# lcp29/trimesh-ray-optix

Measured on AMD Instinct MI355X. Metric: Mrays/s closest-hit, 1M-tri mesh, 1024^2 ray batch, higher is better.
Workload: dtype f32; 1 GPU; C5(i): icosphere(8)+displacement seed 0, 1310720 tris; 1024x1024 pinhole rays per GPU; intersects_closest (stream_compaction=False); rays_per_gpu=1048576, rays_total=1048576, triangles=1310720, parallelism=ray-sharded x1, BVH replicated, warmup_steps_done=368, bvh_depth=30, bvh_bytes=104857568

## Files before the change

### include/triro_hip.h

```cpp
#ifndef TRIRO_HIP_H
#define TRIRO_HIP_H

#include <stdint.h>

#ifdef __cplusplus
extern "C" {
#endif

#define TR_ABI_VERSION 10
#define TR_MAX_ANYHIT_SIZE 8
#define TR_MAX_SIZE_LENGTH 4
#define TR_MAX_HITS_CAP 32

typedef enum tr_status {
    TR_OK = 0,
    TR_ERR_INVALID_ARG = 1,
    TR_ERR_HIP = 2,
    TR_ERR_NO_DEVICE = 3,
    TR_ERR_OUT_OF_MEMORY = 4,
    TR_ERR_INTERNAL = 5
} tr_status;

typedef struct tr_bvh tr_bvh;

// ... 55 lines not shown
int tr_bvh_serialize(const tr_bvh *bvh, void *h_buffer, int64_t size, void *stream);
int tr_bvh_deserialize(const void *h_buffer, int64_t size, void *stream, tr_bvh **out);
int tr_bvh_get_info(const tr_bvh *bvh, tr_bvh_info *info);
int tr_bvh_last_launch(const tr_bvh *bvh, tr_launch_info *info);

typedef struct tr_topology {
    int32_t num_cus, num_xcd, waves_per_cu, reserved;
    int64_t l2_bytes;
    int64_t resident_lanes;
    int64_t steal_max_rays, wide_min_rays, count_stream_min_rays;
} tr_topology;
int tr_device_topology(int device, tr_topology *out);
int tr_bvh_download(const tr_bvh *bvh, void *h_nodes, void *h_links, void *h_tris,
                    void *stream);
int tr_bvh_download_qnodes(const tr_bvh *bvh, void *h_qnodes, float *h_frame6, void *stream);

int tr_intersects_any(const tr_bvh *bvh, const tr_rays *rays, uint8_t *d_hit, void *stream);
int tr_intersects_first(const tr_bvh *bvh, const tr_rays *rays, int32_t *d_tri, void *stream);
int tr_intersects_closest(const tr_bvh *bvh, const tr_rays *rays, uint8_t *d_hit,
                          uint8_t *d_front, int32_t *d_tri, float *d_loc, float *d_uv,
                          void *stream);
int tr_intersects_count(const tr_bvh *bvh, const tr_rays *rays, int32_t *d_count, void *stream);

typedef struct tr_packed_hit {
    uint32_t tri;
    float w0, w1;
} tr_packed_hit;
int tr_intersects_closest_packed(const tr_bvh *bvh, const tr_rays *rays, tr_packed_hit *d_packed,
                                 void *stream);
int tr_closest_expand(const tr_packed_hit *d_packed, int64_t n, const float *d_vertices, int64_t nv,
// ... 54 lines not shown
```

### trimesh-ray-optix_amd/csrc/api.hip

```cpp
#include <atomic>
#include <mutex>
#include <string.h>

#include "tr_internal.h"

namespace {
thread_local std::string g_last_error;
std::mutex g_mutex;
constexpr int TR_MAX_DEVICES = 64;
tr_device_state g_devices[TR_MAX_DEVICES];

struct opt_desc {
    const char* name;
    int tr_options::*field;
    int64_t lo, hi;
    bool boolean;
};
const opt_desc OPTS[] = {
    {"adaptive", &tr_options::adaptive, 0, 1, true},
    {"compact", &tr_options::compact, 0, 1, true},
    {"xcd_chunk", &tr_options::xcd_chunk, 0, 65536, false},
    {"steal", &tr_options::steal, 0, 4096, false},
    {"tile", &tr_options::tile, 0, 2, false},
    {"tile_small", &tr_options::tile_small, 0, 4, false},
// ... 250 lines not shown
    if (hipGetDevice(&device) != hipSuccess)
        return tr_fail(TR_ERR_NO_DEVICE, "no HIP device available (libtriro_hip has no CPU fallback)");
    tr_device_state* st;
    TR_TRY(tr_get_device_state(device, &st));
    tr_bvh* bvh = handle_new(device);
    if (!bvh) return tr_fail(TR_ERR_OUT_OF_MEMORY, "host allocation failed");
    int s = tr_build_impl(bvh, nullptr, 0, nullptr, 0, (hipStream_t)stream);
    if (s == TR_OK && h.num_tris > 0) {
        s = tr_arena_alloc(bvh, h.num_tris);
        if (s == TR_OK && tr_arena_used_bytes(h.num_tris) != h.arena_bytes) s = tr_fail(TR_ERR_INVALID_ARG, "arena size mismatch");
        if (s == TR_OK) {
            if (hipMemcpyAsync(bvh->arena, (const char*)h_buffer + sizeof h, (size_t)h.arena_bytes, hipMemcpyHostToDevice, (hipStream_t)stream) != hipSuccess ||
                hipStreamSynchronize((hipStream_t)stream) != hipSuccess)
                s = tr_fail(TR_ERR_HIP, "upload of the BVH arena failed");
        }
        if (s == TR_OK) {
            bvh->num_tris = h.num_tris; bvh->num_nodes = h.num_nodes; bvh->depth = h.depth; bvh->key_mode = h.key_mode;
            for (int k = 0; k < 3; k++) { bvh->aabb_min[k] = h.aabb_min[k]; bvh->aabb_max[k] = h.aabb_max[k]; }
            tr_qframe_make(bvh->aabb_min, bvh->aabb_max, &bvh->frame);
            s = tr_bvh_sync_frame(bvh);
        }
    }
    if (s != TR_OK) return handle_discard(bvh, s);
    *out = bvh;
    return TR_OK;
}

int tr_bvh_destroy(tr_bvh* bvh) {
    if (!bvh) return TR_OK;
    int status = TR_OK;
    {
        tr_device_guard g;
        if (g.enter(bvh->device) == TR_OK) {
            if (bvh->arena && hipFree(bvh->arena) != hipSuccess) status = tr_fail(TR_ERR_HIP, "hipFree(arena)");
            if (bvh->refit_temp && hipFree(bvh->refit_temp) != hipSuccess) status = tr_fail(TR_ERR_HIP, "hipFree(refit_temp)");
            if (bvh->frame_dev && hipFree(bvh->frame_dev) != hipSuccess) status = tr_fail(TR_ERR_HIP, "hipFree(frame_dev)");
            if (bvh->wnodes && hipFree(bvh->wnodes) != hipSuccess) status = tr_fail(TR_ERR_HIP, "hipFree(wnodes)");
            if (bvh->wflag && hipFree(bvh->wflag) != hipSuccess) status = tr_fail(TR_ERR_HIP, "hipFree(wflag)");
            if (bvh->widx && hipFree(bvh->widx) != hipSuccess) status = tr_fail(TR_ERR_HIP, "hipFree(widx)");
            if (bvh->wide_event) (void)hipEventDestroy(bvh->wide_event);
            for (int k = 0; k < TR_SCHED_SLOTS; k++) {
                if (bvh->sched[k].buf && hipFree(bvh->sched[k].buf) != hipSuccess) status = tr_fail(TR_ERR_HIP, "hipFree(sched)");
                if (bvh->sched[k].wspill && hipFree(bvh->sched[k].wspill) != hipSuccess) status = tr_fail(TR_ERR_HIP, "hipFree(wspill)");
            }
        }
    }
    delete bvh->sched_mutex;
    delete bvh;
    return status;
}

// ... 59 lines not shown
}

int tr_bvh_download_qnodes(const tr_bvh* bvh, void* h_qnodes, float* h_frame6, void* stream) {
    if (!bvh) return tr_fail(TR_ERR_INVALID_ARG, "bvh == NULL");
    hipStream_t s = (hipStream_t)stream;
    tr_device_guard g;
    TR_TRY(tr_enter_device(&g, bvh->device));
    if (h_qnodes && bvh->num_nodes)
        TR_HIP_TRY(hipMemcpyAsync(h_qnodes, bvh->qnodes, sizeof(tr_qnode) * (size_t)bvh->num_nodes, hipMemcpyDeviceToHost, s));
    TR_HIP_TRY(hipStreamSynchronize(s));
    if (h_frame6)
        for (int k = 0; k < 3; k++) { h_frame6[k] = bvh->frame.base[k]; h_frame6[3 + k] = bvh->frame.scale[k]; }
    return TR_OK;
}

int tr_bvh_download(const tr_bvh* bvh, void* h_nodes, void* h_links, void* h_tris, void* stream) {
    if (!bvh) return tr_fail(TR_ERR_INVALID_ARG, "bvh == NULL");
    hipStream_t s = (hipStream_t)stream;
    tr_device_guard g;
    TR_TRY(tr_enter_device(&g, bvh->device));
    if (h_nodes && bvh->num_nodes)
        TR_HIP_TRY(hipMemcpyAsync(h_nodes, bvh->nodes, sizeof(tr_node) * (size_t)bvh->num_nodes, hipMemcpyDeviceToHost, s));
    if (h_links && bvh->num_nodes)
        TR_HIP_TRY(hipMemcpyAsync(h_links, bvh->links, sizeof(tr_link) * (size_t)bvh->num_nodes, hipMemcpyDeviceToHost, s));
    if (h_tris && bvh->num_tris)
        TR_HIP_TRY(hipMemcpyAsync(h_tris, bvh->tris, sizeof(tr_tri) * (size_t)bvh->num_tris, hipMemcpyDeviceToHost, s));
    TR_HIP_TRY(hipStreamSynchronize(s));
    return TR_OK;
}

// ... 19 lines not shown
```

### trimesh-ray-optix_amd/csrc/bvh_build.hip

```cpp
#include <string.h>

#include "tr_internal.h"
#include "tr_lbvh.h"

namespace {

constexpr int RS_KPT = 16;
constexpr int RS_TILE = 64 * RS_KPT;
constexpr int RS_WAVES = 4;

__device__ __forceinline__ uint32_t enc_f32(float f) {
    uint32_t b = __float_as_uint(f);
    return (b & 0x80000000u) ? ~b : (b | 0x80000000u);
}
__device__ __forceinline__ float dec_f32(uint32_t e) {
    uint32_t b = (e & 0x80000000u) ? (e & 0x7fffffffu) : ~e;
    return __uint_as_float(b);
}

__global__ void k_init_bounds(uint32_t* bounds) {
    int t = threadIdx.x;
    if (t < 3) bounds[t] = 0xffffffffu;
    else if (t < 6) bounds[t] = 0u;
    else if (t == 6) bounds[6] = 0xffffffffu;
// ... 260 lines not shown
__global__ void k_qframe(const uint32_t* __restrict__ bounds, tr_qframe* __restrict__ frame) {
    if (threadIdx.x != 0 || blockIdx.x != 0) return;
    float mn[3], mx[3];
    for (int k = 0; k < 3; k++) { mn[k] = dec_f32(bounds[k]); mx[k] = dec_f32(bounds[3 + k]); }
    tr_qframe f;
    tr_qframe_make(mn, mx, &f);
    *frame = f;
}
__global__ void k_qframe_box(const float* __restrict__ box, tr_qframe* __restrict__ frame) {
    if (threadIdx.x != 0 || blockIdx.x != 0) return;
    tr_qframe f;
    tr_qframe_make(box, box + 3, &f);
    *frame = f;
}

__global__ __launch_bounds__(256) void k_emit(const int32_t* __restrict__ childL,
                                              const int32_t* __restrict__ childR,
                                              const int32_t* __restrict__ parent,
                                              const float* __restrict__ sbox,
                                              const float* __restrict__ ibox, int64_t ninternal,
                                              const tr_qframe* __restrict__ frame,
                                              const int32_t* __restrict__ pos,
                                              tr_node* __restrict__ nodes,
                                              tr_link* __restrict__ links,
                                              tr_qnode* __restrict__ qnodes) {
    int64_t i = (int64_t)blockIdx.x * blockDim.x + threadIdx.x;
    if (i >= ninternal) return;
    int32_t cl = childL[i], cr = childR[i];
    const float* a = cl < 0 ? sbox + 6 * (int64_t)(~cl) : ibox + 6 * (int64_t)cl;
    const float* b = cr < 0 ? sbox + 6 * (int64_t)(~cr) : ibox + 6 * (int64_t)cr;
    tr_node nd;
    tr_node_set_box(nd.box0, a, a + 3);
    tr_node_set_box(nd.box1, b, b + 3);
    int32_t p = parent[i];
    int32_t sib = 0;
    if (p >= 0) sib = (childL[p] == (int32_t)i) ? childR[p] : childL[p];
    if (pos && pos[i] < 0) return;
    if (pos) {
        if (cl >= 0) cl = pos[cl];
        if (cr >= 0) cr = pos[cr];
        if (p >= 0) { if (sib >= 0) sib = pos[sib]; p = pos[p]; }
// ... 50 lines not shown
    const float* b = cr < 0 ? sbox + 6 * (int64_t)(~cr) : ibox + 6 * (int64_t)cr;
    float* o = ibox + 6 * i;
#pragma unroll
    for (int k = 0; k < 3; k++) {
        o[k] = fminf(a[k], b[k]);
        o[3 + k] = fmaxf(a[3 + k], b[3 + k]);
    }
    ready[i] = round;
}

__global__ __launch_bounds__(256) void k_update_boxes(tr_node* __restrict__ nodes,
                                                      const float* __restrict__ sbox,
                                                      const float* __restrict__ ibox,
                                                      int64_t ninternal,
                                                      const tr_qframe* __restrict__ frame,
                                                      tr_qnode* __restrict__ qnodes) {
    int64_t i = (int64_t)blockIdx.x * blockDim.x + threadIdx.x;
    if (i >= ninternal) return;
    const int32_t cl = nodes[i].c0, cr = nodes[i].c1;
    const float* a = cl < 0 ? sbox + 6 * (int64_t)(~cl) : ibox + 6 * (int64_t)cl;
    const float* b = cr < 0 ? sbox + 6 * (int64_t)(~cr) : ibox + 6 * (int64_t)cr;
    tr_node_set_box(nodes[i].box0, a, a + 3);
    tr_node_set_box(nodes[i].box1, b, b + 3);
    const tr_qframe f = *frame;
    tr_qnode_set_box(qnodes[i].q, a, a + 3, f);
    tr_qnode_set_box(qnodes[i].q + 3, b, b + 3, f);
}

inline int64_t cdiv(int64_t a, int64_t b) { return (a + b - 1) / b; }
inline size_t align_up(size_t x, size_t a) { return (x + a - 1) / a * a; }

struct Carver {
// ... 26 lines not shown
        TR_HIP_TRY(hipMalloc(&fresh, bytes));
        if (bvh->arena) (void)hipFree(bvh->arena);
        bvh->arena = fresh;
        bvh->arena_bytes = (int64_t)bytes;
        bvh->capacity_tris = nf;
    }
    carve_arena(bvh, (char*)bvh->arena, nf);
    return TR_OK;
}

int64_t tr_arena_used_bytes(int64_t nf) { return (int64_t)carve_arena(nullptr, nullptr, nf); }

int tr_bvh_sync_frame(tr_bvh* bvh) {
    if (!bvh->frame_dev) TR_HIP_TRY(hipMalloc((void**)&bvh->frame_dev, sizeof(tr_qframe)));
    TR_HIP_TRY(hipMemcpy(bvh->frame_dev, &bvh->frame, sizeof(tr_qframe), hipMemcpyHostToDevice));
    return TR_OK;
}

void tr_bvh_reset(tr_bvh* bvh) {
    bvh->wide_valid = false; bvh->wide_unavailable = false;
    bvh->frame = tr_qframe{{0.f, 0.f, 0.f}, {1.f, 1.f, 1.f}};
    bvh->num_tris = 0; bvh->num_nodes = 0; bvh->depth = 0; bvh->key_mode = 0;
    for (int k = 0; k < 3; k++) { bvh->aabb_min[k] = 0.f; bvh->aabb_max[k] = 0.f; }
    for (int k = 0; k < TR_SCHED_SLOTS; k++) { bvh->sched[k].nblocks = 0; }
}

constexpr int TB = 256;
constexpr uint32_t NO_FACE = 0xffffffffu;

static void check(int* status, hipError_t e, const char* what) {
// ... 115 lines not shown
    int32_t root_ready = 0;
    int32_t round = 0;
    const int32_t max_rounds = 160;
    int32_t batch = guess;
    while (root_ready == 0 && round < max_rounds && *status == TR_OK) {
        for (int k = 0; k < batch; k++) {
            ++round;
            hipLaunchKernelGGL(k_refit_round, dim3(gI), dim3(TB), 0, stream, t.cl, t.cr, t.sbox, t.ibox, t.ready, ni, round);
        }
        check(status, hipGetLastError(), "k_refit_round");
        if (!lay_joined) { check(status, hipStreamWaitEvent(stream, st->build_join, 0), "join layout"); lay_joined = true; }
        while (treelets && lround * TR_TREELET_LEVELS < round + TR_TREELET_LEVELS) {
            ++lround;
            hipLaunchKernelGGL(k_layout_round, dim3(gI), dim3(TB), 0, stream, t.cl, t.cr, t.span, t.lpos, t.lbase, t.lflag, ni, lround);
        }
        hipLaunchKernelGGL(k_emit, dim3(gI), dim3(TB), 0, stream, t.cl, t.cr, t.par, t.sbox, t.ibox, ni, t.frame,
                           treelets ? t.lpos : nullptr, bvh->nodes, bvh->links, bvh->qnodes);
        check(status, hipGetLastError(), "k_emit");
        check(status, hipMemcpyAsync(&root_ready, t.ready, sizeof(int32_t), hipMemcpyDeviceToHost, stream), "memcpy root");
        check(status, hipStreamSynchronize(stream), "sync refit");
        if (*bad_face != NO_FACE) return 0;
        batch = 8;
    }
    return root_ready;
}

static void build_hierarchy(tr_bvh* bvh, tr_device_state* st, const build_temps& t, int64_t nf, bool treelets,
                            const uint32_t* bad_face, hipStream_t stream, int* status) {
    int32_t guess = bvh->depth > 0 ? bvh->depth + 1 : 10;
    if (bvh->depth <= 0) for (int64_t m = 1; m < nf; m <<= 1) ++guess;
    if (guess > 64) guess = 64;
    bvh->depth = 0;
// ... 4 lines not shown
        bvh->depth = height;
        bvh->key_mode = mode;
        if (height <= 64) return;
        if (mode == 1) *status = tr_fail(TR_ERR_INTERNAL, "tree height > 64 with bounded keys");
    }
}

int tr_build_impl(tr_bvh* bvh, const float* d_vertices, int64_t nv, const int32_t* d_faces,
                  int64_t nf, hipStream_t stream) {
    if (nf < 0 || nv < 0) return tr_fail(TR_ERR_INVALID_ARG, "negative mesh size");
    if (nf >= (int64_t)1 << 31) return tr_fail(TR_ERR_INVALID_ARG, "more than 2^31-1 triangles");
    bvh->wide_valid = false; bvh->wide_unavailable = false;
    if (nf > 0 && (!d_faces || (!d_vertices && nv > 0))) return tr_fail(TR_ERR_INVALID_ARG, "null mesh pointer");

    int status = tr_arena_alloc(bvh, nf);
    if (status == TR_OK) {
        bvh->num_tris = nf;
        bvh->num_nodes = nf >= 2 ? nf - 1 : 0;
        bvh->depth = 0;
        bvh->key_mode = 0;
        for (int k = 0; k < TR_SCHED_SLOTS; k++) { bvh->sched[k].launches = 0; }
        for (int k = 0; k < 3; k++) { bvh->aabb_min[k] = 0.f; bvh->aabb_max[k] = 0.f; }
    }
    tr_device_state* st = nullptr;
    build_temps t;
    void* temp = nullptr;
    if (status == TR_OK && nf > 0) status = tr_get_device_state(bvh->device, &st);
    if (status == TR_OK && nf > 0) status = tr_build_temp_acquire(st, carve_build_temps(&t, nullptr, nf), &temp);
    if (status == TR_OK && nf > 0) {
        carve_build_temps(&t, (char*)temp, nf);
// ... 54 lines not shown
    }
    carve_refit_temps(&t, (char*)bvh->refit_temp, nf, ni);
    tr_qframe* d_frame = reinterpret_cast<tr_qframe*>(t.bad + 4);
    uint32_t hbad = NO_FACE;
    int status = TR_OK;
    check(&status, hipMemsetAsync(t.bad, 0xff, sizeof(uint32_t), stream), "memset bad-face word");
    hipLaunchKernelGGL(k_regather, dim3((unsigned)cdiv(nf, TB)), dim3(TB), 0, stream, d_vertices, nv, d_faces, nf, bvh->tris, t.sbox, t.bad);
    check(&status, hipGetLastError(), "k_regather");
    check(&status, hipMemcpyAsync(&hbad, t.bad, sizeof(uint32_t), hipMemcpyDeviceToHost, stream), "memcpy bad-face word");
    if (ni > 0) {
        const unsigned gI = (unsigned)cdiv(ni, TB);
        check(&status, hipMemsetAsync(t.ready, 0, sizeof(int32_t) * (size_t)ni, stream), "memset ready");
        for (int32_t round = 1; round <= bvh->depth; round++)
            hipLaunchKernelGGL(k_refit_nodes_round, dim3(gI), dim3(TB), 0, stream, bvh->nodes, t.sbox, t.ibox, t.ready, ni, round);
        hipLaunchKernelGGL(k_qframe_box, dim3(1), dim3(64), 0, stream, t.ibox, d_frame);
        hipLaunchKernelGGL(k_update_boxes, dim3(gI), dim3(TB), 0, stream, bvh->nodes, t.sbox, t.ibox, ni, d_frame, bvh->qnodes);
        check(&status, hipGetLastError(), "refit rounds");
    }
    float box[6];
    check(&status, hipMemcpyAsync(box, ni > 0 ? t.ibox : t.sbox, sizeof(box), hipMemcpyDeviceToHost, stream),
          ni > 0 ? "memcpy root box" : "memcpy box");
    check(&status, hipStreamSynchronize(stream), "sync refit");
    if (status == TR_OK) status = set_bounds(bvh, box, box + 3);
    if (status == TR_OK && hbad != NO_FACE) status = bad_face(hbad, nv);
    return status == TR_OK ? TR_OK : fail_reset(bvh, status);
}
```

### trimesh-ray-optix_amd/csrc/kernels_direct.inc

```
template <bool C, bool DEEP = false> struct tr_word { typedef uint64_t T; };
template <> struct tr_word<true, false> { typedef uint32_t T; };

constexpr bool TR_STREAM_QN = true;
template <int Q> constexpr bool TR_STREAM_COLD = Q != TR_Q_CLOSEST;
template <int Q, int K, bool STATS, bool COMPACT = false, bool UNI = false, bool DEEP = false>
__device__ __forceinline__ void wave_traverse(const tr_bvh_view& b, tr_ray& r, bool go,
                                              tr_result& res, tr_topk<K>& top, tr_counters* cnt,
                                              const tr_ring ring) {
    tr_result_init(res);
    if (Q == TR_Q_LOCATION) top.init();
    typedef typename tr_word<COMPACT, DEEP>::T W;
    tr_state_t<W> fs;
    tr_state_init(fs);
    if (!go) fs.node = -1;
    while (!tr_done(fs)) {
        tr_fused_step<Q, K, STATS, COMPACT, W, UNI, true>(b, r, fs, res, top, cnt, ring);
        TR_CONVERGE();
        tr_fused_step<Q, K, STATS, COMPACT, W, UNI, false>(b, r, fs, res, top, cnt, ring);
        TR_CONVERGE();
    }
}

constexpr uint32_t TR_STEAL_EVERY = 3u;
constexpr uint32_t TR_STEAL_EARLY = 4u;
// ... 74 lines not shown
    if constexpr (PLAIN) {
        bool l0 = false, l1 = false;
        int32_t c0 = 0, c1 = 0;
        bool stop = false;
        {
            const unsigned long long act = __ballot(go);
            if (act != 0ull && trip < steal_min) {
                const int first = (int)__builtin_ctzll(act);
                const uint32_t sn = (uint32_t)__builtin_amdgcn_readlane((int)r.sel_n, first);
                const uint32_t sf = (uint32_t)__builtin_amdgcn_readlane((int)r.sel_f, first);
                const uint32_t sz = (uint32_t)__builtin_amdgcn_readlane((int)r.sel_z, first);
                if (__ballot(go && (r.sel_n != sn || r.sel_f != sf || r.sel_z != sz)) == 0ull) {
                    const tr_uoctant oct = tr_uniform_octant(sn, sz);
                    int32_t nu = 0;
                    tr_uwave u;
                    bool more;
#pragma unroll 1
                    do {
                        typedef const __attribute__((address_space(4))) int32_t* tr_ci32p;
                        const tr_ci32p sp = (tr_ci32p)(unsigned long long)tr_qnode_ptr<COMPACT>(b, nu);
                        tr_i4 w0, w1;
                        w0.x = sp[0]; w0.y = sp[1]; w0.z = sp[2]; w0.w = sp[3];
                        w1.x = sp[4]; w1.y = sp[5]; w1.z = sp[6]; w1.w = sp[7];
                        bool a0, a1, lt;
                        tr_uniform_test<Q>(r, w0, w1, oct, res, a0, a1, lt);
                        if (STATS && go) cnt->nodes++;
                        u = tr_uniform_wave(act, __builtin_amdgcn_ballot_w64(a0), __builtin_amdgcn_ballot_w64(a1),
                                            __builtin_amdgcn_ballot_w64(lt), w1.z, w1.w);
                        c0 = w1.z; c1 = w1.w;
                        if (tr_lane_in(u.both, lane)) tr_addr_push(ar, fs.sa, tr_lane_in(u.sw, lane) ? c0 : c1);
                        TR_CONVERGE();
                        trip++;
                        more = ((u.l0 | u.l1 | u.pop) == 0ull) & ((u.sw == 0ull) | (u.sw == act)) & (trip < steal_min);
                        nu = u.sw != 0ull ? c1 : c0;
                    } while (more);
                    l0 = tr_lane_in(u.l0, lane); l1 = tr_lane_in(u.l1, lane);
                    if (go) fs.node = tr_lane_in(u.sw, lane) ? c1 : c0;
                    if (tr_lane_in(u.pop, lane)) fs.node = tr_addr_pop(ar, fs.sa);
                    stop = (u.l0 | u.l1) != 0ull || !TR_WAVE_ANY(fs.node >= 0);
                }
            }
        }
        if (!stop) while (trip < steal_min) {
            l0 = false; l1 = false;
            if (fs.node >= 0) tr_descent_step<Q, STATS, COMPACT>(b, r, fs, res, cnt, ring, l0, l1, c0, c1);
            TR_CONVERGE();
            trip++;
            if (TR_WAVE_ANY(l0 || l1) || !TR_WAVE_ANY(fs.node >= 0)) break;
        }
        fs.p0 = l0 ? ~c0 : (l1 ? ~c1 : -1);
// ... 705 lines not shown
```

### trimesh-ray-optix_amd/csrc/tr_bvh.h

```cpp
#pragma once
#include <type_traits>
#include "tr_math.h"
#include "../../include/triro_hip.h"

struct alignas(16) tr_f4 {
    float x, y, z, w;
};
struct alignas(16) tr_i4 {
    int32_t x, y, z, w;
};

struct alignas(64) tr_node {
    float box0[6];
    float box1[6];
    int32_t c0, c1;
    int32_t parent;
    int32_t sibling;
};
static_assert(sizeof(tr_node) == 64, "node must be 64 B");
TR_HD void tr_node_set_box(float* box, const float* lo, const float* hi) {
    box[0] = lo[0]; box[1] = lo[1]; box[2] = lo[2]; box[3] = hi[2]; box[4] = hi[0]; box[5] = hi[1];
}

struct alignas(8) tr_link {
// ... 110 lines not shown
    float ax, ay, az, bx, by, bz, cx, cy, cz;
    int32_t face;
    float esum;
    int32_t pad1;
};
static_assert(sizeof(tr_tri) == 48, "tri record must be 48 B");

struct tr_bvh_view {
    const tr_node* nodes;
    const tr_link* links;
    const tr_tri* tris;
    int64_t num_tris;
    const tr_qnode* qnodes;
    tr_qframe frame;
    const tr_qframe* frame_dev;
};
#if defined(__HIP_DEVICE_COMPILE__)
#define TR_VIEW_LIVE(b) do { if ((b).frame_dev) (b).frame = *(b).frame_dev; } while (0)
#else
#define TR_VIEW_LIVE(b) ((void)0)
#endif
enum tr_query { TR_Q_ANY = 0, TR_Q_FIRST = 1, TR_Q_CLOSEST = 2, TR_Q_COUNT = 3, TR_Q_LOCATION = 4 };

struct tr_counters {
    uint32_t nodes, tris, climbs;
};

template <int K>
struct tr_topk {
    float t[K];
// ... 726 lines not shown
    u.l1 = m1 ^ h1;
    u.both = h0 & h1;
    u.sw = ((u.both & lt) | ~h0) & act;
    u.pop = act & ~(h0 | h1);
    return u;
}
TR_HD bool tr_lane_in(uint64_t mask, int lane) {
#if defined(__HIP_DEVICE_COMPILE__)
    (void)lane;
    return __builtin_amdgcn_inverse_ballot_w64(mask);
#else
    return ((mask >> lane) & 1ull) != 0ull;
#endif
}


constexpr int TR_LEAFQ = 6;
struct tr_leafq {
    int32_t* base;
    int32_t stride;
};

template <typename W>
struct tr_ustate_t {
    int32_t node;
    uint32_t depth;
    W trail, owned;
    int32_t nq;
    int32_t pe;
};
// ... 108 lines not shown
```

### trimesh-ray-optix_amd/csrc/tr_internal.h

```cpp
#pragma once
#include <hip/hip_runtime.h>
#include <stdint.h>
#include <mutex>
#include <string>

#include "../../include/triro_hip.h"
#include "tr_bvh.h"
#include "tr_wide.h"

void tr_set_error(const std::string& msg);
int tr_fail(int code, const std::string& msg);

#define TR_HIP_TRY(expr)                                                                  \
    do {                                                                                  \
        hipError_t _e = (expr);                                                           \
        if (_e != hipSuccess) {                                                           \
            return tr_fail(_e == hipErrorOutOfMemory ? TR_ERR_OUT_OF_MEMORY : TR_ERR_HIP, \
                           std::string(#expr) + ": " + hipGetErrorName(_e) + " (" +       \
                               hipGetErrorString(_e) + ")");                              \
        }                                                                                 \
    } while (0)

#define TR_TRY(expr)            \
    do {                        \
// ... 26 lines not shown
struct tr_bvh {
    int device = 0;
    int64_t num_tris = 0;
    int64_t num_nodes = 0;
    int32_t depth = 0;
    int32_t key_mode = 0;
    void* arena = nullptr;
    int64_t arena_bytes = 0;
    int64_t capacity_tris = 0;
    tr_node* nodes = nullptr;
    tr_link* links = nullptr;
    tr_tri* tris = nullptr;
    tr_qnode* qnodes = nullptr;
    tr_qframe frame = {{0, 0, 0}, {1, 1, 1}};
    tr_qframe* frame_dev = nullptr;
    float aabb_min[3] = {0, 0, 0};
    float aabb_max[3] = {0, 0, 0};
    void* refit_temp = nullptr;
    size_t refit_temp_bytes = 0;
    tr_sched_slot sched[TR_SCHED_SLOTS];
    std::mutex* sched_mutex = nullptr;
    tr_wnode* wnodes = nullptr;
    int64_t wcap = 0, wcount = 0;
    uint8_t* wflag = nullptr;
    int64_t* widx = nullptr;
    int64_t wtmp_cap = 0;
    bool wide_valid = false;
    bool wide_unavailable = false;
    hipEvent_t wide_event = nullptr;
    hipStream_t wide_stream = nullptr;
    tr_launch_info last_launch = {};
    bool have_last_launch = false;
};

inline tr_bvh_view tr_view_of(const tr_bvh* bvh) {
    tr_bvh_view view;
    view.nodes = bvh->nodes; view.links = bvh->links; view.tris = bvh->tris; view.num_tris = bvh->num_tris;
    view.qnodes = bvh->qnodes; view.frame = bvh->frame; view.frame_dev = bvh->frame_dev;
    return view;
}

int tr_bvh_sync_frame(tr_bvh* bvh);

struct tr_device_state {
    bool ready = false;
    int device = 0;
    int num_cus = 0;
    int num_xcd = 8;
    int64_t l2_bytes = 0;
    int waves_per_cu = 0;
    int* counters = nullptr;
    unsigned next_counter = 0;
    void* build_temp = nullptr;
    size_t build_temp_bytes = 0;
    std::mutex build_mutex;
// ... 87 lines not shown
```

### trimesh-ray-optix_amd/triro/backend/ops.py

```python
from __future__ import annotations

import ctypes as C
import os
from typing import Tuple

import torch

_INT64_MAX = (1 << 63) - 1
MAX_ANYHIT_SIZE = 8
MAX_SIZE_LENGTH = 4

_LIB_NAME = "libtriro_hip.so"
ABI_VERSION = 10
_lib = None
_lib_error = None


class TrRays(C.Structure):
    _fields_ = [("d_origins", C.c_void_p), ("d_directions", C.c_void_p), ("nray", C.c_int64),
                ("shape", C.c_int64 * 4), ("ostride", C.c_int64 * 4), ("dstride", C.c_int64 * 4)]


class TrTopology(C.Structure):
    _fields_ = [("num_cus", C.c_int32), ("num_xcd", C.c_int32), ("waves_per_cu", C.c_int32), ("reserved", C.c_int32),
# ... 34 lines not shown
    "tr_abi_version": (_int, []),
    "tr_last_error": (C.c_char_p, []),
    "tr_bvh_build": (_int, [_vp, _i64, _vp, _i64, _vp, C.POINTER(_vp)]),
    "tr_bvh_update": (_int, [_vp, _vp, _i64, _vp, _i64, _vp]),
    "tr_bvh_refit": (_int, [_vp, _vp, _i64, _vp, _i64, _vp]),
    "tr_bvh_destroy": (_int, [_vp]),
    "tr_bvh_serialized_size": (_i64, [_vp]),
    "tr_bvh_serialize": (_int, [_vp, _vp, _i64, _vp]),
    "tr_bvh_deserialize": (_int, [_vp, _i64, _vp, C.POINTER(_vp)]),
    "tr_bvh_get_info": (_int, [_vp, C.POINTER(TrBvhInfo)]),
    "tr_bvh_last_launch": (_int, [_vp, C.POINTER(TrLaunchInfo)]),
    "tr_device_topology": (_int, [_int, C.POINTER(TrTopology)]),
    "tr_bvh_replica_hash": (_int, [_vp, C.POINTER(C.c_uint64), _vp]),
    "tr_bvh_download": (_int, [_vp, _vp, _vp, _vp, _vp]),
    "tr_bvh_download_qnodes": (_int, [_vp, _vp, _vp, _vp]),
    "tr_intersects_any": (_int, [_vp, C.POINTER(TrRays), _vp, _vp]),
    "tr_intersects_first": (_int, [_vp, C.POINTER(TrRays), _vp, _vp]),
    "tr_intersects_closest": (_int, [_vp, C.POINTER(TrRays), _vp, _vp, _vp, _vp, _vp, _vp]),
    "tr_intersects_count": (_int, [_vp, C.POINTER(TrRays), _vp, _vp]),
    "tr_intersects_closest_packed": (_int, [_vp, C.POINTER(TrRays), _vp, _vp]),
    "tr_closest_expand": (_int, [_vp, _i64, _vp, _i64, _vp, _i64, _vp, _vp, _vp, _vp, _vp, _vp]),
    "tr_intersects_closest_packed_slots": (_int, [_vp, C.POINTER(TrRays), _vp, _vp]),
    "tr_closest_expand_slots": (_int, [_vp, _vp, _i64, _vp, _vp, _vp, _vp, _vp, _vp]),
    "tr_closest_expand_slots_rows": (_int, [_vp, _vp, _i64, _i64, _vp, _vp, _vp, _vp, _vp, _vp]),
    "tr_intersects_closest_slots": (_int, [_vp, C.POINTER(TrRays), _vp, _vp]),
    "tr_closest_from_slots": (_int, [_vp, C.POINTER(TrRays), _vp, _i64, _vp, _vp, _vp, _vp, _vp, _vp]),
    "tr_hits_scan": (_int, [_vp, _i64, _i32, _vp, _vp, C.POINTER(_i64), _vp]),
    "tr_intersects_location_fill": (_int, [_vp, C.POINTER(TrRays), _i32, _vp, _vp, _vp, _vp, _i64, _vp]),
    "tr_intersects_count_topk": (_int, [_vp, C.POINTER(TrRays), _i32, _vp, _vp, _vp]),
    "tr_location_fill_slots": (_int, [_vp, C.POINTER(TrRays), _i32, _vp, _vp, _vp, _vp, _vp, _vp, _i64, _vp]),
# ... 979 lines not shown
```

### trimesh-ray-optix_amd/triro/ray/ray_optix.py

```python
from __future__ import annotations

import ctypes as C
import os
import warnings
from typing import Optional, Tuple

import numpy as np
import torch

import triro.backend.ops as hops


_points_warned = False


def _default_device() -> torch.device:
    if not torch.cuda.is_available():
        raise RuntimeError("triro (MI355X build) needs a ROCm GPU: torch.cuda.is_available() is False "
                           "and there is no CPU fallback")
    return torch.device("cuda", torch.cuda.current_device())


def _to_device_tensor(x, dtype, device=None) -> torch.Tensor:
    if isinstance(x, torch.Tensor):
# ... 610 lines not shown
        inf = hops.TrBvhInfo()
        hops._check(hops.get_module().tr_bvh_get_info(self._inner, C.byref(inf)))
        return dict(device=inf.device, num_tris=inf.num_tris, num_nodes=inf.num_nodes, depth=inf.depth,
                    key_mode=inf.key_mode, arena_bytes=inf.arena_bytes, node_bytes=inf.node_bytes,
                    tri_bytes=inf.tri_bytes, aabb_min=list(inf.aabb_min), aabb_max=list(inf.aabb_max))

    def download_qnodes(self):
        inf = self.info()
        qn = np.zeros((inf["num_nodes"], 8), np.uint32)
        frame = np.zeros(6, np.float32)
        with torch.cuda.device(inf["device"]):
            stream = torch.cuda.current_stream().cuda_stream
            hops._check(hops.get_module().tr_bvh_download_qnodes(self._inner, qn.ctypes.data, frame.ctypes.data, stream))
        return qn, frame

    def download(self):
        inf = self.info()
        nodes = np.zeros((inf["num_nodes"], 16), np.uint32)
        links = np.zeros((inf["num_nodes"], 2), np.int32)
        tris = np.zeros((inf["num_tris"], 12), np.uint32)
        with torch.cuda.device(inf["device"]):
            stream = torch.cuda.current_stream().cuda_stream
            hops._check(hops.get_module().tr_bvh_download(self._inner, nodes.ctypes.data, links.ctypes.data,
                                                          tris.ctypes.data, stream))
        return nodes, links, tris
```

Before: 8168 Mrays/s.

## Add per-octant float-decoded top-level BVH table for uniform-wave descent

```diff
diff --git a/include/triro_hip.h b/include/triro_hip.h
--- a/include/triro_hip.h
+++ b/include/triro_hip.h
@@ -93,6 +93,9 @@
 int tr_bvh_download(const tr_bvh *bvh, void *h_nodes, void *h_links, void *h_tris,
                     void *stream);
 int tr_bvh_download_qnodes(const tr_bvh *bvh, void *h_qnodes, float *h_frame6, void *stream);
+int tr_bvh_download_top(const tr_bvh *bvh, void *h_top, int32_t *levels, void *stream);
+int tr_bvh_set_float_top(tr_bvh *bvh, int on);
+int tr_bvh_poke_top(tr_bvh *bvh, int64_t slot, const float *h_planes12, void *stream);
 
 int tr_intersects_any(const tr_bvh *bvh, const tr_rays *rays, uint8_t *d_hit, void *stream);
 int tr_intersects_first(const tr_bvh *bvh, const tr_rays *rays, int32_t *d_tri, void *stream);
diff --git a/trimesh-ray-optix_amd/csrc/api.hip b/trimesh-ray-optix_amd/csrc/api.hip
--- a/trimesh-ray-optix_amd/csrc/api.hip
+++ b/trimesh-ray-optix_amd/csrc/api.hip
@@ -288,6 +288,9 @@
                 hipStreamSynchronize((hipStream_t)stream) != hipSuccess)
                 s = tr_fail(TR_ERR_HIP, "upload of the BVH arena failed");
         }
+        if (s == TR_OK && h.num_nodes > 0)
+            s = tr_top_upload(bvh, (const char*)h_buffer + sizeof h + ((const char*)bvh->qnodes - (const char*)bvh->arena),
+                              h.num_nodes, (hipStream_t)stream);
         if (s == TR_OK) {
             bvh->num_tris = h.num_tris; bvh->num_nodes = h.num_nodes; bvh->depth = h.depth; bvh->key_mode = h.key_mode;
             for (int k = 0; k < 3; k++) { bvh->aabb_min[k] = h.aabb_min[k]; bvh->aabb_max[k] = h.aabb_max[k]; }
@@ -309,6 +312,7 @@
             if (bvh->arena && hipFree(bvh->arena) != hipSuccess) status = tr_fail(TR_ERR_HIP, "hipFree(arena)");
             if (bvh->refit_temp && hipFree(bvh->refit_temp) != hipSuccess) status = tr_fail(TR_ERR_HIP, "hipFree(refit_temp)");
             if (bvh->frame_dev && hipFree(bvh->frame_dev) != hipSuccess) status = tr_fail(TR_ERR_HIP, "hipFree(frame_dev)");
+            if (bvh->top && hipFree(bvh->top) != hipSuccess) status = tr_fail(TR_ERR_HIP, "hipFree(top)");
             if (bvh->wnodes && hipFree(bvh->wnodes) != hipSuccess) status = tr_fail(TR_ERR_HIP, "hipFree(wnodes)");
             if (bvh->wflag && hipFree(bvh->wflag) != hipSuccess) status = tr_fail(TR_ERR_HIP, "hipFree(wflag)");
             if (bvh->widx && hipFree(bvh->widx) != hipSuccess) status = tr_fail(TR_ERR_HIP, "hipFree(widx)");
@@ -398,6 +402,37 @@
     return TR_OK;
 }
 
+int tr_bvh_download_top(const tr_bvh* bvh, void* h_top, int32_t* levels, void* stream) {
+    if (!bvh) return tr_fail(TR_ERR_INVALID_ARG, "bvh == NULL");
+    hipStream_t s = (hipStream_t)stream;
+    tr_device_guard g;
+    TR_TRY(tr_enter_device(&g, bvh->device));
+    if (levels) *levels = bvh->top && bvh->num_tris >= 2 ? TR_TOP_LEVELS : 0;
+    if (h_top && bvh->top && bvh->num_tris >= 2)
+        TR_HIP_TRY(hipMemcpyAsync(h_top, bvh->top, sizeof(tr_top_rec) * 8 * (size_t)TR_TOP_SLOTS, hipMemcpyDeviceToHost, s));
+    TR_HIP_TRY(hipStreamSynchronize(s));
+    return TR_OK;
+}
+
+int tr_bvh_poke_top(tr_bvh* bvh, int64_t slot, const float* h_planes12, void* stream) {
+    if (!bvh || !h_planes12) return tr_fail(TR_ERR_INVALID_ARG, "null argument");
+    if (!bvh->top || bvh->num_tris < 2) return tr_fail(TR_ERR_INVALID_ARG, "the handle has no float top");
+    if (slot < 0 || slot >= (int64_t)TR_TOP_SLOTS) return tr_fail(TR_ERR_INVALID_ARG, "slot outside the table");
+    hipStream_t s = (hipStream_t)stream;
+    tr_device_guard g;
+    TR_TRY(tr_enter_device(&g, bvh->device));
+    for (size_t o = 0; o < 8; o++)
+        TR_HIP_TRY(hipMemcpyAsync(bvh->top + o * TR_TOP_SLOTS + (size_t)slot, h_planes12, sizeof(float) * 12, hipMemcpyHostToDevice, s));
+    TR_HIP_TRY(hipStreamSynchronize(s));
+    return TR_OK;
+}
+
+int tr_bvh_set_float_top(tr_bvh* bvh, int on) {
+    if (!bvh) return tr_fail(TR_ERR_INVALID_ARG, "bvh == NULL");
+    bvh->use_top = on != 0;
+    return TR_OK;
+}
+
 int tr_bvh_download(const tr_bvh* bvh, void* h_nodes, void* h_links, void* h_tris, void* stream) {
     if (!bvh) return tr_fail(TR_ERR_INVALID_ARG, "bvh == NULL");
     hipStream_t s = (hipStream_t)stream;
diff --git a/trimesh-ray-optix_amd/csrc/bvh_build.hip b/trimesh-ray-optix_amd/csrc/bvh_build.hip
--- a/trimesh-ray-optix_amd/csrc/bvh_build.hip
+++ b/trimesh-ray-optix_amd/csrc/bvh_build.hip
@@ -1,4 +1,5 @@
 #include <string.h>
+#include <vector>
 
 #include "tr_internal.h"
 #include "tr_lbvh.h"
@@ -298,6 +299,26 @@
     *frame = f;
 }
 
+template <typename Kids>
+__device__ void top_slot_emit(tr_top_rec* __restrict__ top, uint32_t slot, Kids kids, const int32_t* __restrict__ pos,
+                              const float* __restrict__ sbox, const float* __restrict__ ibox, const tr_qframe* __restrict__ frame) {
+    int32_t n = tr_top_walk(slot, kids);
+    if (n >= 0 && pos && pos[n] < 0) n = -1;
+    tr_qnode qn;
+    if (n >= 0) {
+        int32_t cl, cr;
+        kids(n, cl, cr);
+        const float* a = cl < 0 ? sbox + 6 * (int64_t)(~cl) : ibox + 6 * (int64_t)cl;
+        const float* b = cr < 0 ? sbox + 6 * (int64_t)(~cr) : ibox + 6 * (int64_t)cr;
+        const tr_qframe f = *frame;
+        tr_qnode_set_box(qn.q, a, a + 3, f);
+        tr_qnode_set_box(qn.q + 3, b, b + 3, f);
+        qn.c0 = (pos && cl >= 0) ? pos[cl] : cl;
+        qn.c1 = (pos && cr >= 0) ? pos[cr] : cr;
+    }
+    tr_top_write_slot(top, n >= 0 ? &qn : nullptr, slot, TR_TOP_SLOTS);
+}
+
 __global__ __launch_bounds__(256) void k_emit(const int32_t* __restrict__ childL,
                                               const int32_t* __restrict__ childR,
                                               const int32_t* __restrict__ parent,
@@ -307,8 +328,11 @@
                                               const int32_t* __restrict__ pos,
                                               tr_node* __restrict__ nodes,
                                               tr_link* __restrict__ links,
-                                              tr_qnode* __restrict__ qnodes) {
+                                              tr_qnode* __restrict__ qnodes,
+                                              tr_top_rec* __restrict__ top) {
     int64_t i = (int64_t)blockIdx.x * blockDim.x + threadIdx.x;
+    if (top && i < (int64_t)TR_TOP_SLOTS)
+        top_slot_emit(top, (uint32_t)i, [=](int32_t n, int32_t& c0, int32_t& c1) { c0 = childL[n]; c1 = childR[n]; }, pos, sbox, ibox, frame);
     if (i >= ninternal) return;
     int32_t cl = childL[i], cr = childR[i];
     const float* a = cl < 0 ? sbox + 6 * (int64_t)(~cl) : ibox + 6 * (int64_t)cl;
@@ -389,8 +413,11 @@
                                                       const float* __restrict__ ibox,
                                                       int64_t ninternal,
                                                       const tr_qframe* __restrict__ frame,
-                                                      tr_qnode* __restrict__ qnodes) {
+                                                      tr_qnode* __restrict__ qnodes,
+                                                      tr_top_rec* __restrict__ top) {
     int64_t i = (int64_t)blockIdx.x * blockDim.x + threadIdx.x;
+    if (top && i < (int64_t)TR_TOP_SLOTS)
+        top_slot_emit(top, (uint32_t)i, [=](int32_t n, int32_t& c0, int32_t& c1) { c0 = nodes[n].c0; c1 = nodes[n].c1; }, nullptr, sbox, ibox, frame);
     if (i >= ninternal) return;
     const int32_t cl = nodes[i].c0, cr = nodes[i].c1;
     const float* a = cl < 0 ? sbox + 6 * (int64_t)(~cl) : ibox + 6 * (int64_t)cl;
@@ -447,6 +474,31 @@
 int tr_bvh_sync_frame(tr_bvh* bvh) {
     if (!bvh->frame_dev) TR_HIP_TRY(hipMalloc((void**)&bvh->frame_dev, sizeof(tr_qframe)));
     TR_HIP_TRY(hipMemcpy(bvh->frame_dev, &bvh->frame, sizeof(tr_qframe), hipMemcpyHostToDevice));
+    return TR_OK;
+}
+
+int tr_top_alloc(tr_bvh* bvh) {
+    if (!bvh->top) TR_HIP_TRY(hipMalloc((void**)&bvh->top, sizeof(tr_top_rec) * 8 * (size_t)TR_TOP_SLOTS));
+    return TR_OK;
+}
+
+int tr_top_upload(tr_bvh* bvh, const void* h_qnodes, int64_t num_nodes, hipStream_t stream) {
+    if (num_nodes < 1) return TR_OK;
+    TR_TRY(tr_top_alloc(bvh));
+    std::vector<tr_top_rec> host((size_t)8 * TR_TOP_SLOTS);
+    auto fetch = [&](int32_t node) { tr_qnode q; memcpy(&q, (const char*)h_qnodes + sizeof(tr_qnode) * (size_t)node, sizeof q); return q; };
+    for (uint32_t s = 0; s < TR_TOP_SLOTS; s++) {
+        const int32_t node = tr_top_walk(s, [&](int32_t n, int32_t& c0, int32_t& c1) {
+            const tr_qnode q = fetch(n);
+            c0 = q.c0 < num_nodes ? q.c0 : -1;
+            c1 = q.c1 < num_nodes ? q.c1 : -1;
+        });
+        tr_qnode q;
+        if (node >= 0) q = fetch(node);
+        tr_top_write_slot(host.data(), node >= 0 ? &q : nullptr, s, TR_TOP_SLOTS);
+    }
+    TR_HIP_TRY(hipMemcpyAsync(bvh->top, host.data(), sizeof(tr_top_rec) * host.size(), hipMemcpyHostToDevice, stream));
+    TR_HIP_TRY(hipStreamSynchronize(stream));
     return TR_OK;
 }
 
@@ -592,8 +644,9 @@
             ++lround;
             hipLaunchKernelGGL(k_layout_round, dim3(gI), dim3(TB), 0, stream, t.cl, t.cr, t.span, t.lpos, t.lbase, t.lflag, ni, lround);
         }
-        hipLaunchKernelGGL(k_emit, dim3(gI), dim3(TB), 0, stream, t.cl, t.cr, t.par, t.sbox, t.ibox, ni, t.frame,
-                           treelets ? t.lpos : nullptr, bvh->nodes, bvh->links, bvh->qnodes);
+        const unsigned gE = (unsigned)cdiv(ni > (int64_t)TR_TOP_SLOTS ? ni : (int64_t)TR_TOP_SLOTS, TB);
+        hipLaunchKernelGGL(k_emit, dim3(gE), dim3(TB), 0, stream, t.cl, t.cr, t.par, t.sbox, t.ibox, ni, t.frame,
+                           treelets ? t.lpos : nullptr, bvh->nodes, bvh->links, bvh->qnodes, bvh->top);
         check(status, hipGetLastError(), "k_emit");
         check(status, hipMemcpyAsync(&root_ready, t.ready, sizeof(int32_t), hipMemcpyDeviceToHost, stream), "memcpy root");
         check(status, hipStreamSynchronize(stream), "sync refit");
@@ -628,6 +681,7 @@
     if (nf > 0 && (!d_faces || (!d_vertices && nv > 0))) return tr_fail(TR_ERR_INVALID_ARG, "null mesh pointer");
 
     int status = tr_arena_alloc(bvh, nf);
+    if (status == TR_OK && nf >= 2) status = tr_top_alloc(bvh);
     if (status == TR_OK) {
         bvh->num_tris = nf;
         bvh->num_nodes = nf >= 2 ? nf - 1 : 0;
@@ -712,7 +766,8 @@
         for (int32_t round = 1; round <= bvh->depth; round++)
             hipLaunchKernelGGL(k_refit_nodes_round, dim3(gI), dim3(TB), 0, stream, bvh->nodes, t.sbox, t.ibox, t.ready, ni, round);
         hipLaunchKernelGGL(k_qframe_box, dim3(1), dim3(64), 0, stream, t.ibox, d_frame);
-        hipLaunchKernelGGL(k_update_boxes, dim3(gI), dim3(TB), 0, stream, bvh->nodes, t.sbox, t.ibox, ni, d_frame, bvh->qnodes);
+        const unsigned gE = (unsigned)cdiv(ni > (int64_t)TR_TOP_SLOTS ? ni : (int64_t)TR_TOP_SLOTS, TB);
+        hipLaunchKernelGGL(k_update_boxes, dim3(gE), dim3(TB), 0, stream, bvh->nodes, t.sbox, t.ibox, ni, d_frame, bvh->qnodes, bvh->top);
         check(&status, hipGetLastError(), "refit rounds");
     }
     float box[6];
diff --git a/trimesh-ray-optix_amd/csrc/kernels_direct.inc b/trimesh-ray-optix_amd/csrc/kernels_direct.inc
--- a/trimesh-ray-optix_amd/csrc/kernels_direct.inc
+++ b/trimesh-ray-optix_amd/csrc/kernels_direct.inc
@@ -112,7 +112,39 @@
                     const tr_uoctant oct = tr_uniform_octant(sn, sz);
                     int32_t nu = 0;
                     tr_uwave u;
-                    bool more;
+                    bool more = true;
+                    if (b.top) {
+                        typedef float tr_rec16 __attribute__((ext_vector_type(16)));
+                        typedef const __attribute__((address_space(4))) tr_rec16* tr_crecp;
+                        typedef const __attribute__((address_space(4))) char* tr_cchp;
+                        const tr_cchp tab = (tr_cchp)(unsigned long long)(b.top + tr_octant_index(sn, sz) * TR_TOP_SLOTS);
+                        uint32_t off = 0;
+                        const uint32_t lim = steal_min < trip + TR_TOP_LEVELS ? steal_min : trip + TR_TOP_LEVELS;
+                        int32_t s0, s1;
+                        bool on;
+#pragma unroll 1
+                        do {
+                            const tr_rec16 w = *(tr_crecp)(tab + off);
+                            float p[12];
+#pragma unroll
+                            for (int k = 0; k < 12; k++) p[k] = w[k];
+                            s0 = (int32_t)__float_as_uint(w[12]); s1 = (int32_t)__float_as_uint(w[13]);
+                            bool a0, a1, lt;
+                            tr_top_test<Q>(r, p, res, a0, a1, lt);
+                            if (STATS && go) cnt->nodes++;
+                            u = tr_uniform_wave(act, __builtin_amdgcn_ballot_w64(a0), __builtin_amdgcn_ballot_w64(a1),
+                                                __builtin_amdgcn_ballot_w64(lt), s0, s1);
+                            c0 = s0; c1 = s1;
+                            if (tr_lane_in(u.both, lane)) tr_addr_push(ar, fs.sa, tr_lane_in(u.sw, lane) ? c0 : c1);
+                            TR_CONVERGE();
+                            trip++;
+                            on = ((u.l0 | u.l1 | u.pop) == 0ull) & ((u.sw == 0ull) | (u.sw == act));
+                            off = 2u * off + (u.sw != 0ull ? 128u : 64u);
+                        } while (on & (trip < lim));
+                        more = on & (trip < steal_min);
+                        nu = u.sw != 0ull ? s1 : s0;
+                    }
+                    if (more) {
 #pragma unroll 1
                     do {
                         typedef const __attribute__((address_space(4))) int32_t* tr_ci32p;
@@ -132,6 +164,7 @@
                         more = ((u.l0 | u.l1 | u.pop) == 0ull) & ((u.sw == 0ull) | (u.sw == act)) & (trip < steal_min);
                         nu = u.sw != 0ull ? c1 : c0;
                     } while (more);
+                    }
                     l0 = tr_lane_in(u.l0, lane); l1 = tr_lane_in(u.l1, lane);
                     if (go) fs.node = tr_lane_in(u.sw, lane) ? c1 : c0;
                     if (tr_lane_in(u.pop, lane)) fs.node = tr_addr_pop(ar, fs.sa);
diff --git a/trimesh-ray-optix_amd/csrc/tr_bvh.h b/trimesh-ray-optix_amd/csrc/tr_bvh.h
--- a/trimesh-ray-optix_amd/csrc/tr_bvh.h
+++ b/trimesh-ray-optix_amd/csrc/tr_bvh.h
@@ -148,6 +148,7 @@
     const tr_qnode* qnodes;
     tr_qframe frame;
     const tr_qframe* frame_dev;
+    const struct tr_top_rec* top = nullptr;
 };
 #if defined(__HIP_DEVICE_COMPILE__)
 #define TR_VIEW_LIVE(b) do { if ((b).frame_dev) (b).frame = *(b).frame_dev; } while (0)
@@ -904,6 +905,87 @@
 #endif
 }
 
+#define TR_TOP_LEVELS 12
+#define TR_TOP_SLOTS ((1u << TR_TOP_LEVELS) - 1u)
+struct alignas(64) tr_top_rec {
+    float p[12];
+    int32_t c0, c1;
+    uint32_t pad[2];
+};
+static_assert(sizeof(tr_top_rec) == 64, "a record of the float top is one 64-byte line");
+TR_HD uint32_t tr_octant_index(uint32_t sel_n, uint32_t sel_z) {
+    return ((sel_n & 0x0400u) ? 1u : 0u) | ((sel_n & 0x04000000u) ? 2u : 0u) | ((sel_z & 2u) ? 4u : 0u);
+}
+TR_HD tr_uoctant tr_octant_of_index(uint32_t o) {
+    return tr_uoctant{((o & 1u) ? 0xffffu : 0u) | ((o & 2u) ? 0xffff0000u : 0u), (o & 4u) ? 16u : 0u, (o & 4u) ? 0u : 16u};
+}
+TR_HD void tr_top_fill(tr_top_rec& t, const tr_qnode& n, uint32_t o) {
+    const tr_uoctant oct = tr_octant_of_index(o);
+#pragma unroll
+    for (int c = 0; c < 2; c++) {
+        const uint32_t x = (n.q[3 * c] ^ n.q[3 * c + 2]) & oct.mxy;
+        const uint32_t e = n.q[3 * c] ^ x, f = n.q[3 * c + 2] ^ x, z = n.q[3 * c + 1];
+        t.p[6 * c + 0] = (float)(e & 0xffffu); t.p[6 * c + 1] = (float)(e >> 16);
+        t.p[6 * c + 2] = (float)(f & 0xffffu); t.p[6 * c + 3] = (float)(f >> 16);
+        t.p[6 * c + 4] = (float)((z >> oct.she) & 0xffffu); t.p[6 * c + 5] = (float)((z >> oct.shf) & 0xffffu);
+    }
+    t.c0 = n.c0; t.c1 = n.c1;
+    t.pad[0] = 0u; t.pad[1] = 0u;
+}
+template <int Q, typename P>
+TR_HD void tr_top_test(const tr_ray& r, const P& p, const tr_result& res, bool& a0, bool& a1, bool& lt) {
+    float tn[2], tf[2];
+#pragma unroll
+    for (int c = 0; c < 2; c++) {
+#if defined(__HIP_DEVICE_COMPILE__)
+        typedef float tr_v2 __attribute__((ext_vector_type(2)));
+        const tr_v2 a = __builtin_elementwise_fma(tr_v2{p[6 * c + 0], p[6 * c + 1]}, tr_v2{r.qax, r.qay}, tr_v2{r.qnx, r.qny});
+        const tr_v2 b = __builtin_elementwise_fma(tr_v2{p[6 * c + 2], p[6 * c + 3]}, tr_v2{r.qax, r.qay}, tr_v2{r.qfx, r.qfy});
+        const tr_v2 d = __builtin_elementwise_fma(tr_v2{p[6 * c + 4], p[6 * c + 5]}, tr_v2{r.qaz, r.qaz2}, tr_v2{r.qnz, r.qfz});
+        tn[c] = fmaxf(fmaxf(a.x, a.y), d.x);
+        tf[c] = fminf(fminf(b.x, b.y), d.y);
+#else
+        tn[c] = fmaxf(fmaxf(fmaf(p[6 * c + 0], r.qax, r.qnx), fmaf(p[6 * c + 1], r.qay, r.qny)), fmaf(p[6 * c + 4], r.qaz, r.qnz));
+        tf[c] = fminf(fminf(fmaf(p[6 * c + 2], r.qax, r.qfx), fmaf(p[6 * c + 3], r.qay, r.qfy)), fmaf(p[6 * c + 5], r.qaz, r.qfz));
+#endif
+    }
+    const float lim = tr_cull_limit<Q>(res);
+    a0 = tr_slab_hit(tn[0], tf[0], lim);
+    a1 = tr_slab_hit(tn[1], tf[1], lim);
+    lt = tn[1] < tn[0];
+}
+TR_HD int tr_top_level(uint32_t slot) {
+    int level = 0;
+    while (((slot + 1u) >> (level + 1)) != 0u) level++;
+    return level;
+}
+TR_HD void tr_top_write_slot(tr_top_rec* top, const tr_qnode* qn, uint32_t slot, uint32_t slots) {
+    for (uint32_t o = 0; o < 8u; o++) {
+        tr_top_rec t;
+        if (qn) tr_top_fill(t, *qn, o);
+        else { for (int k = 0; k < 12; k++) t.p[k] = 0.f; t.c0 = 0; t.c1 = 0; t.pad[0] = 0u; t.pad[1] = 0u; }
+        top[(size_t)o * slots + slot] = t;
+    }
+}
+template <typename Kids>
+TR_HD int32_t tr_top_walk(uint32_t slot, Kids kids) {
+    const uint32_t path = slot + 1u;
+    int32_t node = 0;
+    for (int k = tr_top_level(slot) - 1; k >= 0 && node >= 0; k--) {
+        int32_t c0, c1;
+        kids(node, c0, c1);
+        node = ((path >> k) & 1u) ? c1 : c0;
+    }
+    return node;
+}
+TR_HD void tr_top_build_slot(tr_top_rec* top, const tr_qnode* qnodes, int64_t num_nodes, uint32_t slot, uint32_t slots) {
+    const int32_t node = tr_top_walk(slot, [=](int32_t n, int32_t& c0, int32_t& c1) {
+        c0 = qnodes[n].c0 < num_nodes ? qnodes[n].c0 : -1;
+        c1 = qnodes[n].c1 < num_nodes ? qnodes[n].c1 : -1;
+    });
+    tr_top_write_slot(top, node >= 0 ? qnodes + node : nullptr, slot, slots);
+}
+
 
 constexpr int TR_LEAFQ = 6;
 struct tr_leafq {
diff --git a/trimesh-ray-optix_amd/csrc/tr_internal.h b/trimesh-ray-optix_amd/csrc/tr_internal.h
--- a/trimesh-ray-optix_amd/csrc/tr_internal.h
+++ b/trimesh-ray-optix_amd/csrc/tr_internal.h
@@ -64,6 +64,8 @@
     tr_qnode* qnodes = nullptr;
     tr_qframe frame = {{0, 0, 0}, {1, 1, 1}};
     tr_qframe* frame_dev = nullptr;
+    tr_top_rec* top = nullptr;
+    bool use_top = true;
     float aabb_min[3] = {0, 0, 0};
     float aabb_max[3] = {0, 0, 0};
     void* refit_temp = nullptr;
@@ -87,8 +89,12 @@
     tr_bvh_view view;
     view.nodes = bvh->nodes; view.links = bvh->links; view.tris = bvh->tris; view.num_tris = bvh->num_tris;
     view.qnodes = bvh->qnodes; view.frame = bvh->frame; view.frame_dev = bvh->frame_dev;
+    view.top = bvh->num_tris >= 2 && bvh->use_top ? bvh->top : nullptr;
     return view;
 }
+
+int tr_top_alloc(tr_bvh* bvh);
+int tr_top_upload(tr_bvh* bvh, const void* h_qnodes, int64_t num_nodes, hipStream_t stream);
 
 int tr_bvh_sync_frame(tr_bvh* bvh);
 
diff --git a/trimesh-ray-optix_amd/triro/backend/ops.py b/trimesh-ray-optix_amd/triro/backend/ops.py
--- a/trimesh-ray-optix_amd/triro/backend/ops.py
+++ b/trimesh-ray-optix_amd/triro/backend/ops.py
@@ -72,6 +72,9 @@
     "tr_bvh_replica_hash": (_int, [_vp, C.POINTER(C.c_uint64), _vp]),
     "tr_bvh_download": (_int, [_vp, _vp, _vp, _vp, _vp]),
     "tr_bvh_download_qnodes": (_int, [_vp, _vp, _vp, _vp]),
+    "tr_bvh_download_top": (_int, [_vp, _vp, _vp, _vp]),
+    "tr_bvh_set_float_top": (_int, [_vp, _int]),
+    "tr_bvh_poke_top": (_int, [_vp, C.c_int64, _vp, _vp]),
     "tr_intersects_any": (_int, [_vp, C.POINTER(TrRays), _vp, _vp]),
     "tr_intersects_first": (_int, [_vp, C.POINTER(TrRays), _vp, _vp]),
     "tr_intersects_closest": (_int, [_vp, C.POINTER(TrRays), _vp, _vp, _vp, _vp, _vp, _vp]),
diff --git a/trimesh-ray-optix_amd/triro/ray/ray_optix.py b/trimesh-ray-optix_amd/triro/ray/ray_optix.py
--- a/trimesh-ray-optix_amd/triro/ray/ray_optix.py
+++ b/trimesh-ray-optix_amd/triro/ray/ray_optix.py
@@ -648,6 +648,27 @@
             hops._check(hops.get_module().tr_bvh_download_qnodes(self._inner, qn.ctypes.data, frame.ctypes.data, stream))
         return qn, frame
 
+    def set_float_top(self, on: bool):
+        hops._check(hops.get_module().tr_bvh_set_float_top(self._inner, int(bool(on))))
+
+    def poke_top(self, slot: int, planes12):
+        p = np.ascontiguousarray(planes12, np.float32).reshape(12)
+        with torch.cuda.device(self.info()["device"]):
+            hops._check(hops.get_module().tr_bvh_poke_top(self._inner, int(slot), p.ctypes.data, torch.cuda.current_stream().cuda_stream))
+
+    def download_top(self):
+        inf = self.info()
+        levels = C.c_int32(0)
+        with torch.cuda.device(inf["device"]):
+            stream = torch.cuda.current_stream().cuda_stream
+            lib = hops.get_module()
+            hops._check(lib.tr_bvh_download_top(self._inner, None, C.byref(levels), stream))
+            if levels.value == 0:
+                return None
+            top = np.zeros((8, (1 << levels.value) - 1, 64), np.uint8)
+            hops._check(lib.tr_bvh_download_top(self._inner, top.ctypes.data, None, stream))
+        return top
+
     def download(self):
         inf = self.info()
         nodes = np.zeros((inf["num_nodes"], 16), np.uint32)
```

New measurement: 8482 Mrays/s, median of 6. 3.8% higher.
